# Amelie-Schreiber/ShapeMol

Measured on AMD Instinct MI355X. Metric: molecules/sec (1000-step DDPM sample, batch 256), higher is better.
Workload: dtype f32 (matrix operands split exactly into 3 x bf16 pieces = 24 bits, six piece products, fp32 accumulate); 1 GPU; BASELINE configs[1]: batch 256 MOSES-prior molecules (9-27 atoms) per GPU, 1000-step chain, fp32 results, k=8, synthetic shapes + hash-filled weights; besides the 5 warm-up steps an untimed 200-step chain runs first to reach the loaded clocks; batch_per_gpu=256, atoms_per_gpu=5541, total_atoms=5541, noise=device Philox, trajectories=kept in HBM, launch=hipGraph replay, parallelism=dp1 (whole batches per rank), ranks_seen=1

## Files before the change

### shapemol_amd/csrc/shapemol_hip.hip

```cpp
#include "../../include/shapemol_hip.h"
#include "sm_device.h"
#include "sm_edge.h"
#include "sm_edge_bf16.h"
#include "sm_edge16.h"
#include "sm_node.h"
#include "sm_node16.h"
#include "sm_edge_stream.h"
#include "sm_misc.h"
#include "sm_mesh.h"
#include "sm_guide_groups.h"
#include "sm_cfg.h"
#include "sm_mesh_groups.h"
#include <hip/hip_ext.h>

#include <algorithm>
#include <cmath>
#include <type_traits>
#include <cstdio>
#include <cstring>
#include <map>
#include <string>
#include <vector>

#include "sm_pack.h"

namespace {

#define HIPCHK(expr)                                                                         \
    do {                                                                                     \
        hipError_t e_ = (expr);                                                              \
        if (e_ != hipSuccess)                                                                \
            return fail(std::string(#expr) + ": " + hipGetErrorString(e_));                  \
    } while (0)

constexpr int kEdgeThreadsDefault = 768;
#ifndef SM_GRAPH_UNROLL
#define SM_GRAPH_UNROLL 20
#endif
constexpr int kGraphUnroll = SM_GRAPH_UNROLL;

struct ProfRec { const char *name; hipEvent_t e0, e1; };

enum class Guide { None, Cloud, Groups, Mesh, MeshGroups, Cfg };

}

struct shapemol_ctx {
    shapemol_config cfg{};
    int device = 0;
    int KP = 8;
    float *d_img = nullptr;
    float *ttab = nullptr;
    float *etab = nullptr;
    DevModel dm;
    int64_t capN = 0, capB = 0;
    std::vector<void *> allocs;
    int *mol_of = nullptr, *mol_off = nullptr, *t_mol = nullptr, *nbr = nullptr, *steps = nullptr;
    float *temb = nullptr, *inv = nullptr, *add0 = nullptr, *addp = nullptr, *ps = nullptr, *ew = nullptr;
    float *h_a = nullptr, *h_b = nullptr, *pre0 = nullptr, *preAB = nullptr, *q_x = nullptr, *q_h = nullptr, *att = nullptr, *o3 = nullptr, *pd = nullptr;
    ShapeTermArgs *prep_terms = nullptr; VnShapeArgs *prep_vn = nullptr; int n_prep_terms = 0;
    int2 *mol_span = nullptr;
    float *xsum = nullptr;
    float *part_rows = nullptr, *part_ms = nullptr;
    float *alpha = nullptr;
    float *x_a = nullptr, *x_b = nullptr, *x_state = nullptr, *pred_pos = nullptr, *pred_v = nullptr;
    int64_t *v_state = nullptr;
    unsigned long long *stamps = nullptr;
    unsigned long long *kstamps = nullptr;
    int kstamp_sel = -1;
    int stamp_on = 0;
    double *bn_acc = nullptr;
    int *status = nullptr;
    ChainParams *chain_params = nullptr;
    int64_t lastN = 0, lastB = 0;
    const float *last_h = nullptr, *last_x = nullptr;
    int stop_layer = -1, edge_threads = 0 , lin_waves = 16, edge_bf16 = 2, lin_bf16 = 1, chain_bf16 = 1, vn_fuse = 2;
    int vn_fold = 1;
    int max_mol_atoms = 0;
    int stream_whole_rounds = 0;
    int lin_fuse = 0;
    int bn_eval = 0;
    float *bn_run = nullptr;
    double *bn_eval_acc = nullptr;
    int ddpm_fold = 1;
    DdpmFold ddpm_vf{};
    int graph_fuse = 1;
// ... 445 lines not shown
               bool half_tiles, unsigned long long *stamps) {
    a.pre = pre; a.ld_pre = ld_pre; a.q = q; a.x = x; a.nbr = c->nbr; a.ew = c->ew; a.out = out; a.n_atoms = n_atoms; a.stamps = stamps;
    if (half_tiles) { a.out = c->part_rows; a.part_ms = c->part_ms; }
}

EdgeFusedArgs::VnFuse vn_fuse_args(const shapemol_ctx *c, int l, float *x_next, unsigned *arrive, int enable) {
    const DevLayer &D = c->dm.layer[l];
    const int hd = c->cfg.n_heads;
    return {c->ps + (size_t)l * c->capB * 2 * hd * 3, c->P(D.wf_x), c->P(D.wd_x), c->P(D.wf_o), c->P(D.wd_o), c->P(D.bn_g), c->P(D.bn_b),
            c->mol_of, c->pd, c->bn_acc + (size_t)l * kBnReplicas * 2 * hd, arrive, c->status + ST_VN_BARRIER, x_next, enable};
}

struct H2xPlan { EdgeFusedArgs::VnFuse vn{}; float *xsum = nullptr; VnFold pending{}; DdpmFold ddpm{}; bool stats_done = false, vn_done = false; };
H2xPlan h2x_plan(const shapemol_ctx *c, int l, bool fold, bool has_next, bool half_tiles, const double *stat_acc, const float *cur_x,
                 float *x_next, float *out_pos) {
    H2xPlan p;
    if (!c->vn_fuse || half_tiles) return p;
    const DevLayer &D = c->dm.layer[l];
    const int hd = c->cfg.n_heads;
    const double *acc = stat_acc + (size_t)l * kBnReplicas * 2 * hd;
    p.vn = vn_fuse_args(c, l, x_next, nullptr, 2);
    p.stats_done = true;
    const bool to_ddpm = !has_next && l == c->cfg.num_layers - 1 && out_pos && c->ddpm_fold && chain_guide(c) == Guide::None &&
                         c->cfg.num_classes <= 16 && hd <= 16;
    if (fold && has_next) p.pending = VnFold{c->pd, acc, c->P(D.bn_g), c->P(D.bn_b), c->xsum, cur_x, x_next, c->mol_span, c->status + ST_SPAN, 1};
    else if (fold && to_ddpm) p.ddpm = DdpmFold{c->pd, acc, c->P(D.bn_g), c->P(D.bn_b), c->xsum, cur_x, out_pos, hd, 1};
    else return p;
    p.xsum = c->xsum;
    p.vn_done = true;
    return p;
}

template <int H>
int run_score(shapemol_ctx *c, hipStream_t s, const float *x_in, const int64_t *v_in, int64_t N, int64_t B,
              bool sampling, int t_first, float *out_pos, float *out_h, float *out_v, bool reuse_graph = false) {
    const shapemol_config &g = c->cfg;
    const int L = g.num_layers, hd = g.n_heads, C = g.num_classes, D = g.time_emb_dim, KP = c->KP;
    const int n = (int)N;
    AtomEmbArgs ae{c->P(c->dm.embw), c->P(c->dm.embb), v_in, c->mol_of, c->ttab, c->t_mol, sampling ? c->steps : nullptr,
                   c->steps + 1, c->bn_acc, c->h_a, n, H, C, D, t_first, L * kBnReplicas * 2 * hd + L};
    const int nlay = c->stop_layer >= 0 ? std::min(c->stop_layer, L) : L;
    const bool fused_prologue = c->chain_bf16 && c->lin_bf16;
    if (fused_prologue) {
        const DevLayer &D0 = c->dm.layer[0];
        NodePrologueArgs pa{};
        pa.emb_wT = c->P(c->dm.embwT); pa.emb_b = ae.b; pa.v = v_in; pa.mol_of = c->mol_of; pa.ttab = c->ttab; pa.etab = c->etab; pa.t_mol = c->t_mol;
        pa.step_ptr = ae.step_ptr; pa.step_cur = ae.step_cur; pa.bn_acc = c->bn_acc; pa.h_out = c->h_a;
        pa.q = follow_of(c, D0.q_x2h, NODE_LN_RELU, c->q_x, H, H);
        pa.lin_img6 = c->P(c->node_f16 ? D0.pre16_x2h : D0.pre6_x2h); pa.add_mol = c->add0; pa.pre_out = c->pre0;
        pa.n_lin_tiles = nlay > 0 ? 4 * (H / 16) : 0; pa.ld_add = 4 * H; pa.ld_out = 4 * H;
        pa.n_atoms = n; pa.C = C; pa.D = D; pa.t_first = t_first; pa.bn_acc_len = ae.bn_acc_len;
        pa.stamps = c->kstamp_sel == 5 ? c->kstamps : nullptr;
        const int n_ct = (n + 15) / 16;
        if (c->node_f16 && c->feat_f16) LAUNCH("node_prologue", SMK((node_prologue16_kernel<H, true>), dim3((n_ct + CHAIN_COLS - 1) / CHAIN_COLS), dim3(H * 4),
                                                   2 * Chain16Lds<H>::FRAG * 16 + Chain16Lds<H>::PRE * 4, s, pa, c->status + ST_RANGE));
        else if (c->node_f16) LAUNCH("node_prologue", SMK(node_prologue16_kernel<H>, dim3((n_ct + CHAIN_COLS - 1) / CHAIN_COLS), dim3(H * 4),
                                                   2 * Chain16Lds<H>::FRAG * 16 + Chain16Lds<H>::PRE * 4, s, pa, c->status + ST_RANGE));
        else LAUNCH("node_prologue", SMK(node_prologue6_kernel<H>, dim3((n_ct + CHAIN_COLS - 1) / CHAIN_COLS), dim3(H * 4),
                                                   2 * Chain6Lds<H>::FRAG * 16 + Chain6Lds<H>::PRE * 4, s, pa));
    } else {
        LAUNCH("embed", SMK(atom_embed_kernel, dim3((N * H + 255) / 256), dim3(256), 0, s, ae));
    }
    const bool graph_fused = sampling && c->graph_fuse && c->max_mol_atoms > 0 && c->max_mol_atoms <= kGraphCap && KP <= 32 && c->n_pins == 0;
    if (reuse_graph) {
    } else if (graph_fused) {
        GraphArgs ga{x_in, c->mol_span, n, g.knn, KP, c->nbr, c->P(c->dm.ew.w1), c->P(c->dm.ew.b1), c->P(c->dm.ew.g), c->P(c->dm.ew.be),
                     c->P(c->dm.ew.w2), c->P(c->dm.ew.b2), c->ew, c->status + ST_SPAN, c->kstamp_sel == 4 ? c->kstamps : nullptr};
        const int apb = kGraphWaves * (KP >= 16 ? 1 : 16 / KP);
        DISPATCH_KP("graph", graph_kernel, (), dim3((n + apb - 1) / apb), dim3(kGraphWaves * 64), 0, s, ga);
    } else LAUNCH("knn", SMK(knn_kernel, dim3((N + 3) / 4), dim3(256), 0, s, x_in, c->mol_of, c->mol_off, n, g.knn, KP, c->nbr));
    if (sampling && c->n_pins > 0 && !reuse_graph)
        LAUNCH("knn", SMK(knn_pin_kernel, dim3(32), dim3(256), 0, s, c->pin_off, c->pin_steps, c->pin_atom, c->pin_nbr, c->pin_k, KP, c->steps + 1, n, c->nbr));
    EdgeWeightArgs ea{x_in, c->nbr, c->P(c->dm.ew.w1), c->P(c->dm.ew.b1), c->P(c->dm.ew.g), c->P(c->dm.ew.be),
                      c->P(c->dm.ew.w2), c->P(c->dm.ew.b2), c->ew, n * KP, KP};
    if (!graph_fused && !reuse_graph) {
        const int tiles = (n * KP + 15) / 16;
        LAUNCH("edge_weight", SMK(edge_weight_kernel<H>, dim3((tiles + 3) / 4), dim3(256), 0, s, ea));
    }
    const float *cur_x = x_in;
    float *cur_h = c->h_a;
    constexpr int NT = H / 16;
    bool v_done = false;
    if (nlay > 0 && !fused_prologue) {
        const DevLayer &D0 = c->dm.layer[0];
        if (launch_linear<H>(c, s, "node_pre", cur_h, c->P(D0.pre_x2h), c->P(D0.pre6_x2h), c->P(D0.pre16_x2h), c->add0, 4 * H, c->pre0, 4 * H, 4 * NT, n,
                             c->kstamp_sel == 0 ? c->kstamps : nullptr)) return 1;
        if (launch_mlp2<H, 1>(c, s, "node_q", D0.q_x2h, cur_h, nullptr, NODE_LN_RELU, nullptr, c->q_x, H, H, n)) return 1;
    }
    const bool fold = sampling && vn_fold_ok(c, n);
    double *stat_acc = c->bn_acc;
    if (c->bn_eval) {
        if (!c->bn_run) return fail("bn_eval = 1 needs the running statistics (shapemol_set_bn_running)");
// ... 181 lines not shown
    c->num_cu = prop.multiProcessorCount > 0 ? prop.multiProcessorCount : 256;

    Image im;
    if (build_model_image(*cfg, hm, im, c->dm, c->hid_max)) { delete c; return 1; }
    const DevModel &dm = c->dm;
    const int H = cfg->hidden_dim, T = cfg->num_timesteps;
    if (hipMalloc((void **)&c->d_img, im.d.size() * sizeof(float)) != hipSuccess) { delete c; return fail("hipMalloc(weights) failed"); }
    if (hipMemcpy(c->d_img, im.d.data(), im.d.size() * sizeof(float), hipMemcpyHostToDevice) != hipSuccess) { hipFree(c->d_img); delete c; return fail("hipMemcpy(weights) failed"); }
    if (H == 128 ? set_edge_attr<128>(c->KP) : set_edge_attr<32>(c->KP)) { hipFree(c->d_img); delete c; return 1; }
    {
        if (hipMalloc((void **)&c->ttab, (size_t)T * cfg->time_emb_dim * sizeof(float)) != hipSuccess) { hipFree(c->d_img); delete c; return fail("hipMalloc(time table) failed"); }
        TimeTableArgs ta{c->P(dm.te1w), c->P(dm.te1b), c->P(dm.te2w), c->P(dm.te2b), c->ttab, T, cfg->time_emb_dim};
        hipLaunchKernelGGL(time_table_kernel, dim3((T + 63) / 64), dim3(64), 0, nullptr, ta);
        if (hipDeviceSynchronize() != hipSuccess) { hipFree(c->ttab); hipFree(c->d_img); delete c; return fail("time table kernel failed"); }
        const int C = cfg->num_classes;
        if (hipMalloc((void **)&c->etab, (size_t)T * C * H * sizeof(float)) != hipSuccess) { hipFree(c->ttab); hipFree(c->d_img); delete c; return fail("hipMalloc(embedding table) failed"); }
        const int items = T * C * (H / 4);
        hipLaunchKernelGGL(emb_table_kernel, dim3((items + 255) / 256), dim3(256), 0, nullptr, c->P(dm.embwT), c->P(dm.embb), c->ttab, c->etab, T, C, cfg->time_emb_dim, H);
        if (hipDeviceSynchronize() != hipSuccess) { hipFree(c->etab); hipFree(c->ttab); hipFree(c->d_img); delete c; return fail("embedding table kernel failed"); }
    }
    *out = c;
    return 0;
}

void shapemol_destroy(shapemol_ctx *c) {
    if (!c) return;
    hipSetDevice(c->device);
    hipDeviceSynchronize();
    c->drop_graphs();
    for (auto &r : c->prof) { hipEventDestroy(r.e0); hipEventDestroy(r.e1); }
    for (void *p : c->allocs) hipFree(p);
    hipFree(c->ttab);
    hipFree(c->etab);
    hipFree(c->d_img);
    if (c->g_cloud) hipFree(c->g_cloud);
    if (c->gg_clouds) hipFree(c->gg_clouds);
    if (c->gg_table) hipFree(c->gg_table);
    if (c->m_faces) hipFree(c->m_faces);
    if (c->mg_faces) hipFree(c->mg_faces);
    if (c->m_within) hipFree(c->m_within);
    if (c->bn_run) hipFree(c->bn_run);
    if (c->bn_eval_acc) hipFree(c->bn_eval_acc);
    if (c->pin_off) { hipFree(c->pin_off); hipFree(c->pin_atom); hipFree(c->pin_nbr); }
    delete c;
}

int shapemol_set_bn_running(shapemol_ctx *c, const float *h_mean, const float *h_var, int64_t count) {
    if (!c || !h_mean || !h_var) return fail("shapemol_set_bn_running: null argument");
    const int L = c->cfg.num_layers, hd = c->cfg.n_heads;
    if (count != (int64_t)L * hd) return fail("shapemol_set_bn_running: count must be num_layers * n_heads");
    for (int64_t i = 0; i < count; ++i)
        if (!(h_var[i] >= 0.f) || !std::isfinite(h_mean[i]) || !std::isfinite(h_var[i])) return fail("shapemol_set_bn_running: statistics must be finite, variance >= 0");
    HIPCHK(hipSetDevice(c->device));
    HIPCHK(hipDeviceSynchronize());
    if (!c->bn_run) {
        HIPCHK(hipMalloc(&c->bn_run, 2 * count * sizeof(float)));
        HIPCHK(hipMalloc(&c->bn_eval_acc, (size_t)L * kBnReplicas * 2 * hd * sizeof(double)));
    }
    HIPCHK(hipMemcpy(c->bn_run, h_mean, count * sizeof(float), hipMemcpyHostToDevice));
    HIPCHK(hipMemcpy(c->bn_run + count, h_var, count * sizeof(float), hipMemcpyHostToDevice));
    return 0;
}

int shapemol_reserve(shapemol_ctx *c, int64_t max_atoms, int64_t max_mols) {
    if (!c || max_atoms < 1 || max_mols < 1) return fail("shapemol_reserve: bad argument");
    return ensure_workspace(c, max_atoms, max_mols);
}

int shapemol_score(shapemol_ctx *c, const float *d_pos, const int64_t *d_v, const int64_t *d_batch, int64_t N,
                   int64_t B, const float *d_shape, const int64_t *d_t, float *out_pos, float *out_h, float *out_v,
                   void *stream) {
    if (!c || !d_pos || !d_v || !d_batch || !d_shape || !d_t || !out_pos || !out_v) return fail("shapemol_score: null argument");
    if (N < 1 || B < 1 || N > (1 << 27)) return fail("shapemol_score: n_atoms / n_mols out of range");
    HIPCHK(hipSetDevice(c->device));
    if (ensure_workspace(c, N, B)) return 1;
    hipStream_t s = (hipStream_t)stream;
    c->lastN = N; c->lastB = B;
    HIPCHK(hipMemsetAsync(c->status, 0, 8 * sizeof(int), s));
    if (DISPATCH_H(c, run_prep<128>(c, s, d_batch, N, B, d_shape), run_prep<32>(c, s, d_batch, N, B, d_shape))) return 1;
    LAUNCH("prep", SMK(t_convert_kernel, dim3((B + 255) / 256), dim3(256), 0, s, d_t, (int)B, c->cfg.num_timesteps, c->t_mol, c->status));
    LAUNCH("prep", SMK(v_check_kernel, dim3((N + 255) / 256), dim3(256), 0, s, d_v, (int)N, c->cfg.num_classes, c->status));
    return DISPATCH_H(c, run_score<128>(c, s, d_pos, d_v, N, B, false, 0, out_pos, out_h, out_v),
                      run_score<32>(c, s, d_pos, d_v, N, B, false, 0, out_pos, out_h, out_v));
}

int shapemol_sample(shapemol_ctx *c, const float *d_init_pos, const int64_t *d_init_v, const int64_t *d_batch,
                    int64_t N, int64_t B, const float *d_shape, int32_t num_steps, const float *d_eps, const float *d_u,
                    uint64_t seed, const shapemol_traj *traj, float *out_pos, int64_t *out_v, int32_t use_graph, void *stream) {
    if (!c || !d_init_pos || !d_init_v || !d_batch || !d_shape || !out_pos || !out_v) return fail("shapemol_sample: null argument");
    if (N < 1 || B < 1 || N > (1 << 27)) return fail("shapemol_sample: n_atoms / n_mols out of range");
    if (num_steps < 1 || c->first_step + num_steps > c->cfg.num_timesteps) return fail("shapemol_sample: num_steps out of range");
    if ((d_eps == nullptr) != (d_u == nullptr)) return fail("shapemol_sample: d_eps and d_u must be given together");
    HIPCHK(hipSetDevice(c->device));
    if (ensure_workspace(c, N, B)) return 1;
    hipStream_t s = (hipStream_t)stream;
    c->lastN = N; c->lastB = B;
    const int t_first = c->cfg.num_timesteps - 1;
    const Guide kind = chain_guide(c);
    const bool mesh = kind == Guide::Mesh, mesh_groups = kind == Guide::MeshGroups, cfg = kind == Guide::Cfg;
    if (mesh && mesh_workspace(c, N, 1)) return 1;
    if (mesh_groups && mesh_workspace(c, N, c->mg_groups)) return 1;
    if (c->mg_groups > 0 && c->mg_mols != B)
        return fail("shapemol_sample: n_mols = " + std::to_string(B) + " but the mesh guidance groups cover " + std::to_string(c->mg_mols) + " molecules");
    if (c->gg_groups > 0 && c->gg_mols != B)
        return fail("shapemol_sample: n_mols = " + std::to_string(B) + " but the guidance groups cover " + std::to_string(c->gg_mols) + " molecules");
    if (kind == Guide::Groups && groups_table(c, s, d_batch, N, c->gg_ints, c->gg_groups)) return 1;
    if (mesh_groups && groups_table(c, s, d_batch, N, c->mg_ints, c->mg_groups)) return 1;
    HIPCHK(hipMemsetAsync(c->status, 0, 8 * sizeof(int), s));
    if (mesh) HIPCHK(hipMemsetAsync(c->m_cnt, 0, 4 * sizeof(int), s));
    if (mesh_groups && mesh_counters_clear(c, s, c->mg_groups)) return 1;
    if (DISPATCH_H(c, run_prep<128>(c, s, d_batch, N, B, d_shape), run_prep<32>(c, s, d_batch, N, B, d_shape))) return 1;
    if (cfg) {
        swap_uncond(c);
        const int rc = DISPATCH_H(c, run_prep_shape<128>(c, s, B, c->shape_zero), run_prep_shape<32>(c, s, B, c->shape_zero));
        swap_uncond(c);
        if (rc) return 1;
        HIPCHK(hipMemsetAsync(c->cfg_hist, 0, (size_t)2 * kCfgHistWords * sizeof(unsigned), s));
    }
    LAUNCH("prep", SMK(v_check_kernel, dim3((N + 255) / 256), dim3(256), 0, s, d_init_v, (int)N, c->cfg.num_classes, c->status));
    {
        ChainParams cp{};
        cp.seed = seed; cp.eps = d_eps; cp.u = d_u; cp.step_base = c->first_step; cp.guide_draws = mesh ? c->m_draws : (mesh_groups ? c->mg_draws : (c->gg_groups > 0 ? c->gg_draws : c->g_draws));
        if (traj) { cp.tr_pos = traj->pos_traj; cp.tr_v = traj->v_traj; cp.tr_v0 = traj->v0_traj; cp.tr_vt = traj->vt_traj;
                    cp.tr_pos_cond = traj->pos_cond_traj; cp.tr_v_cond = traj->v_cond_traj; }
        if (cfg) { cp.tr_pos_uncond = c->cfg_tr_pos_u; cp.tr_v_uncond = c->cfg_tr_v_u; }
        LAUNCH("prep", SMK(set_chain_params_kernel, dim3(1), dim3(1), 0, s, c->chain_params, cp, c->steps));
    }
    HIPCHK(hipMemcpyAsync(c->x_state, d_init_pos, N * 3 * sizeof(float), hipMemcpyDeviceToDevice, s));
    HIPCHK(hipMemcpyAsync(c->v_state, d_init_v, N * sizeof(int64_t), hipMemcpyDeviceToDevice, s));
// ... 65 lines not shown
int shapemol_set_option(shapemol_ctx *c, const char *name, int64_t value) {
    if (!c || !name) return fail("shapemol_set_option: null argument");
    const std::string k(name);
    if (k == "max_mol_atoms") {
        if (value < 0) return fail("max_mol_atoms must be >= 0");
        c->max_mol_atoms = (int)std::min<int64_t>(value, 1 << 20);
        return 0;
    }
    if (k == "first_step") {
        if (value < 0 || value >= c->cfg.num_timesteps) return fail("first_step must be in [0, num_timesteps)");
        c->first_step = (int)value;
        return 0;
    }
    if (k == "stop_layer") c->stop_layer = (int)value;
    else if (k == "edge_bf16") {
        if (value < 0 || value > 3) return fail("edge_bf16 must be 0 (fp32 MFMA), 1 (exactly split bf16, phase kernels), 2 (exactly split bf16, streaming kernels) or 3 (two-piece f16)");
        if (value != 3 && value != 2 && c->KP > 16) return fail("k > 16 runs on the streaming (edge_bf16 = 2) or the two-piece f16 (edge_bf16 = 3) edge kernels");
        if (value == 3 && c->hid_max > 6.0e4f) return fail("edge_bf16 = 3: the edge MLPs' LayerNorm outputs may exceed the fp16 range for these weights");
        c->edge_bf16 = (int)value;
    }
    else if (k == "edge_tiles") { if (value < -1 || value > 1) return fail("edge_tiles must be -1 (automatic), 0 (sliced one-job launches) or 1 (looping launch)"); c->edge_tiles = (int)value; }
    else if (k == "node_f16") c->node_f16 = value != 0;
    else if (k == "feat_f16") {
        if (value && (c->edge_bf16 != 3 || !c->node_f16)) return fail("feat_f16 = 1 needs the f16 kernels (edge_bf16 = 3, node_f16 = 1)");
        c->feat_f16 = value != 0;
    }
    else if (k == "lin_fuse") c->lin_fuse = value != 0;
    else if (k == "stream_whole_rounds") c->stream_whole_rounds = value != 0;
    else if (k == "x2h_chain") c->x2h_chain = value != 0;
    else if (k == "graph_fuse") c->graph_fuse = value != 0;
    else if (k == "bn_eval") c->bn_eval = value != 0;
    else if (k == "ddpm_fold") c->ddpm_fold = value != 0;
    else if (k == "vn_fold") c->vn_fold = value != 0;
    else if (k == "lin_bf16") c->lin_bf16 = (int)value;
    else if (k == "chain_bf16") c->chain_bf16 = (int)value;
    else if (k == "vn_fuse") c->vn_fuse = (int)value;
    else if (k == "lin_waves") { if (value < 1 || value > 16) return fail("lin_waves must be 1..16"); c->lin_waves = (int)value; }
    else if (k == "stamps") c->stamp_on = (int)value;
    else if (k == "kstamp_sel") c->kstamp_sel = (int)value;
    else if (k == "edge_waves") { if (value < 0 || value > 12) return fail("edge_waves must be 0 (automatic) .. 12"); c->edge_threads = (int)value * 64; }
    else return fail("unknown option " + k);
    hipSetDevice(c->device);
    c->drop_graphs();
    return 0;
}

int64_t shapemol_debug_read(shapemol_ctx *c, const char *name, void *dst, size_t max_bytes) {
    if (!c || !name || !dst) { fail("shapemol_debug_read: null argument"); return -1; }
    const std::string k(name);
    const shapemol_config &g = c->cfg;
    const int64_t N = c->lastN;
    const void *src = nullptr; size_t bytes = 0;
    int64_t dims[8] = {N, c->lastB, c->KP, g.hidden_dim, g.n_heads, g.num_layers, c->capN, c->capB};
    if (k == "dims") { if (max_bytes < sizeof(dims)) return -1; std::memcpy(dst, dims, sizeof(dims)); return sizeof(dims); }
    if (k == "captures") { if (max_bytes < 8) return -1; std::memcpy(dst, &c->n_captures, 8); return 8; }
    if (k == "nbr") { src = c->nbr; bytes = N * c->KP * 4; }
    else if (k == "ew") { src = c->ew; bytes = N * c->KP * 4; }
    else if (k == "h") { src = c->last_h; bytes = N * g.hidden_dim * 4; }
    else if (k == "x") { src = c->last_x; bytes = N * 3 * 4; }
    else if (k == "pre") { src = c->preAB; bytes = N * 8 * g.hidden_dim * 4; }
    else if (k == "q") { src = c->q_h; bytes = N * g.hidden_dim * 4; }
    else if (k == "att") { src = c->att; bytes = N * g.hidden_dim * 4; }
    else if (k == "o3") { src = c->o3; bytes = N * 48 * 4; }
    else if (k == "stamps") { src = c->stamps; bytes = 2048 * 8; }
    else if (k == "kstamps") { src = c->kstamps; bytes = (size_t)8 * 16 * 4096 * 8; }
    else if (k == "vn_err") { src = c->status + ST_VN_BARRIER; bytes = 4; }
    else if (k == "mesh_group_flags") { src = c->m_cnt ? c->m_cnt + 4 * c->m_cnt_cap : nullptr; bytes = (size_t)c->mg_flag_groups * 4; }
    else if (k == "cfg_stat") { src = c->cfg_stat; bytes = 2 * 4; }
    else if (k == "bnstat") { src = c->bn_acc; bytes = (size_t)g.num_layers * kBnReplicas * 2 * g.n_heads * 8; }
    else { fail("shapemol_debug_read: unknown buffer " + k); return -1; }
    if (!src || bytes > max_bytes) { fail("shapemol_debug_read: buffer unavailable or destination too small"); return -1; }
    if (hipSetDevice(c->device) != hipSuccess || hipDeviceSynchronize() != hipSuccess ||
        hipMemcpy(dst, src, bytes, hipMemcpyDeviceToHost) != hipSuccess) { fail("shapemol_debug_read: copy failed"); return -1; }
    return (int64_t)bytes;
}

void shapemol_debug_split_exact(float x, uint16_t *pieces) {
    uint16_t p[3];
    split3_host(x, p);
    pieces[0] = p[0]; pieces[1] = p[1]; pieces[2] = p[2];
}

int shapemol_set_knn_pins(shapemol_ctx *c, const int32_t *h_off, int32_t n_steps, const int32_t *h_atom, const int32_t *h_nbr, int64_t n_pins, int32_t k) {
    if (!c) return fail("shapemol_set_knn_pins: null context");
    HIPCHK(hipSetDevice(c->device));
    c->drop_graphs();
    HIPCHK(hipDeviceSynchronize());
    if (c->pin_off) { hipFree(c->pin_off); hipFree(c->pin_atom); hipFree(c->pin_nbr); c->pin_off = c->pin_atom = c->pin_nbr = nullptr; }
    c->n_pins = 0; c->pin_steps = 0; c->pin_k = 0;
    if (n_pins <= 0) return 0;
    if (!h_off || !h_atom || !h_nbr || n_steps < 1 || k < 1 || k > c->KP) return fail("shapemol_set_knn_pins: bad arguments");
    if (h_off[0] != 0 || h_off[n_steps] != n_pins) return fail("shapemol_set_knn_pins: offsets do not cover the pins");
// ... 92 lines not shown
```

### shapemol_amd/csrc/sm_misc.h

```cpp
#pragma once
#include "sm_device.h"
#include "sm_cfg.h"

enum StatusFlag { ST_VN_BARRIER = 0, ST_BATCH = 1, ST_ATOM_TYPE = 2, ST_TIME = 3, ST_RANGE = 4, ST_SPAN = 5, ST_MESH = 6 };

__global__ void mol_index_kernel(const int64_t *batch, int n, int n_mols, int *mol_of, int *mol_off, int *status) {
    const int i = blockIdx.x * blockDim.x + threadIdx.x;
    if (i >= n) return;
    const int64_t braw = batch[i], praw = i == 0 ? -1 : batch[i - 1];
    if (braw < 0 || braw >= n_mols || braw < praw) status[ST_BATCH] = 1;
    const int b = (int)min(max(braw, (int64_t)0), (int64_t)n_mols - 1);
    const int prev = (int)min(max(praw, (int64_t)-1), (int64_t)n_mols - 1);
    mol_of[i] = b;
    for (int m = prev + 1; m <= b; ++m) mol_off[m] = i;
    if (i == n - 1)
        for (int m = b + 1; m <= n_mols; ++m) mol_off[m] = n;
}

__global__ void mol_span_kernel(const int *mol_of, const int *mol_off, int n, int2 *span) {
    const int i = blockIdx.x * blockDim.x + threadIdx.x;
    if (i < n) span[i] = int2{mol_off[mol_of[i]], mol_off[mol_of[i] + 1]};
}

__global__ void t_convert_kernel(const int64_t *t, int n_mols, int n_timesteps, int *t_mol, int *status) {
// ... 184 lines not shown
    for (int k = 0; k < D; ++k) {
        const float4 wk = ldg4(emb_wT + (size_t)(C + k) * H + f);
        const float tk = te[k];
        y[0] += wk.x * tk; y[1] += wk.y * tk; y[2] += wk.z * tk; y[3] += wk.w * tk;
    }
    stg4(etab + ((size_t)t * C + v) * H + f, float4{y[0], y[1], y[2], y[3]});
}

struct AtomEmbArgs {
    const float *w, *b;
    const int64_t *v;
    const int *mol_of;
    const float *ttab;
    const int *t_mol;
    const int *step_ptr;
    int *step_cur;
    double *bn_acc;
    float *h;
    int n_atoms, H, C, D, t_first, bn_acc_len;
};
__global__ void atom_embed_kernel(AtomEmbArgs a) {
    const int idx = blockIdx.x * blockDim.x + threadIdx.x;
    const int step = a.step_ptr ? *a.step_ptr : 0;
    if (idx == 0 && a.step_ptr) *a.step_cur = step;
    for (int i = idx; i < a.bn_acc_len; i += gridDim.x * blockDim.x) a.bn_acc[i] = 0.0;
    if (idx >= a.n_atoms * a.H) return;
    const int i = idx / a.H, f = idx % a.H, ld = a.C + a.D;
    const int t = a.step_ptr ? a.t_first - step : a.t_mol[a.mol_of[i]];
    const float *w = a.w + (size_t)f * ld;
    float y = a.b[f] + w[min(max((int)a.v[i], 0), a.C - 1)];
    const float *te = a.ttab + (size_t)t * a.D;
    for (int k = 0; k < a.D; ++k) y += w[a.C + k] * te[k];
    a.h[idx] = y;
}

SM_DEV float dist2_rounded(float dx, float dy, float dz) {
#pragma clang fp contract(off)
    const float a = dx * dx, b = dy * dy, c = dz * dz;
    return (a + b) + c;
}

__global__ void knn_kernel(const float *x, const int *mol_of, const int *mol_off, int n_atoms, int k,
                           int kp, int *nbr) {
    const int lane = threadIdx.x & 63;
    const int i = blockIdx.x * (blockDim.x >> 6) + (threadIdx.x >> 6);
    if (i >= n_atoms) return;
    const int m = mol_of[i], s = mol_off[m], cnt = mol_off[m + 1] - s;
    const float xi = x[i * 3], yi = x[i * 3 + 1], zi = x[i * 3 + 2];
    const int deg = min(k, cnt - 1);
    for (int c = lane; c < cnt; c += 64) {
        const int j = s + c;
        if (j == i) continue;
        float dx = x[j * 3] - xi, dy = x[j * 3 + 1] - yi, dz = x[j * 3 + 2] - zi;
        const float dc = dist2_rounded(dx, dy, dz);
        int rank = 0;
        for (int o = 0; o < cnt; ++o) {
            const int jo = s + o;
            dx = x[jo * 3] - xi; dy = x[jo * 3 + 1] - yi; dz = x[jo * 3 + 2] - zi;
            const float d_o = dist2_rounded(dx, dy, dz);
            rank += (jo != i) && (o != c) && (d_o < dc || (d_o == dc && o < c));
        }
        if (rank < k) nbr[(size_t)i * kp + rank] = j;
    }
    for (int sl = lane; sl < kp; sl += 64)
        if (sl >= deg) nbr[(size_t)i * kp + sl] = -1;
}
// ... 679 lines not shown
```

### shapemol_amd/csrc/sm_node.h

```cpp
#pragma once
#include "sm_device.h"

enum NodeMode { NODE_LN_RELU = 1, NODE_SSP = 2 };
constexpr int kNodeThreads = 1024;

struct NodeLinArgs {
    const float *in;
    const float *wimg;
    const float *add_mol;
    const int *mol_of;
    float *out;
    int n_atoms, n_out_tiles, tiles_per_group;
    int ld_add, ld_out;
    unsigned long long *stamps;
    int nwave;
};

constexpr int kLinChunk = 8;

template <int H>
__global__ void __launch_bounds__(kNodeThreads)
node_linear_kernel(NodeLinArgs a) {
    constexpr int NT = H / 16;
    constexpr int XS = H + 16;
// ... 706 lines not shown
        const int fa = 32 * sb + 4 * (sl >> 4);
        float vv[8];
        {
            const float *row = a.etab + ((size_t)t * a.C + vi) * H + fa;
            const float4 r0 = ldg4(row), r1 = ldg4(row + 16);
            vv[0] = r0.x; vv[1] = r0.y; vv[2] = r0.z; vv[3] = r0.w; vv[4] = r1.x; vv[5] = r1.y; vv[6] = r1.z; vv[7] = r1.w;
        }
        if (at_raw < a.n_atoms) {
            stg4(a.h_out + (size_t)at * H + fa, float4{vv[0], vv[1], vv[2], vv[3]});
            stg4(a.h_out + (size_t)at * H + fa + 16, float4{vv[4], vv[5], vv[6], vv[7]});
        }
        u32x4 hi, mid, lo;
        split3_bf16(vv, hi, mid, lo);
        u32x4 *dst = fh + (sb * CC + sc) * 64 + frag_slot(sb, sl);
        dst[0] = hi; dst[NB * CC * 64] = mid; dst[2 * NB * CC * 64] = lo;
    }
    if (a.n_lin_tiles > 0) load_w(a.lin_img6, ot, wl);
    const float4 b1 = ldg4(a.q.b1 + f0);
    __syncthreads();

    {
        f32x4 acc[CC];
#pragma unroll
        for (int c = 0; c < CC; ++c) acc[c] = f32x4{b1.x, b1.y, b1.z, b1.w};
        gemm6(wq1, fh, acc);
#pragma unroll
        for (int c = 0; c < CC; ++c) stg4(pre0 + (c * 16 + n) * XS + f0, float4{acc[c][0], acc[c][1], acc[c][2], acc[c][3]});
    }
    const bool onq = ot < a.q.nt2;
    if (onq) load_w(a.q.w2img6, ot, wq1);
    auto lin_tile = [&](int tile, const u32x4 (&w)[3][NB]) {
        f32x4 acc[CC];
#pragma unroll
        for (int c = 0; c < CC; ++c) {
            const float4 t = a.add_mol ? ldg4(a.add_mol + (size_t)a.mol_of[atom_of(c)] * a.ld_add + 16 * tile + 4 * g)
                                       : float4{0.f, 0.f, 0.f, 0.f};
            acc[c] = f32x4{t.x, t.y, t.z, t.w};
        }
        gemm6(w, fh, acc);
#pragma unroll
        for (int c = 0; c < CC; ++c)
            if (atom_ok(c)) stg4(a.pre_out + (size_t)atom_of(c) * a.ld_out + 16 * tile + 4 * g, float4{acc[c][0], acc[c][1], acc[c][2], acc[c][3]});
    };
    for (int tile = ot; tile < a.n_lin_tiles; tile += 2 * NT) {
        u32x4 wn[3][NB];
        const bool more1 = tile + NT < a.n_lin_tiles, more2 = tile + 2 * NT < a.n_lin_tiles;
        if (more1) load_w(a.lin_img6, tile + NT, wn);
        lin_tile(tile, wl);
        if (more2) load_w(a.lin_img6, tile + 2 * NT, wl);
        if (more1) lin_tile(tile + NT, wn);
    }
    __syncthreads();
    {
        const int col = ot * (64 / LPC) + lane / LPC, ln = lane % LPC;
        const int b = ln >> 2, gg = ln & 3;
        const int fa = 32 * b + 4 * gg;
        const float4 p0 = ldg4(pre0 + col * XS + fa), p1 = ldg4(pre0 + col * XS + fa + 16);
        float v[8] = {p0.x, p0.y, p0.z, p0.w, p1.x, p1.y, p1.z, p1.w};
        float s = 0.f;
#pragma unroll
        for (int i = 0; i < 8; ++i) s += v[i];
        const float mean = seg_sum<LPC>(s) * (1.0f / H);
        float q = 0.f;
#pragma unroll
        for (int i = 0; i < 8; ++i) { const float d = v[i] - mean; q += d * d; }
        const float var = seg_sum<LPC>(q) * (1.0f / H);
        const float rstd = 1.0f / sqrtf(var + 1e-5f);
        const float4 g0 = ldg4(a.q.ln_g + fa), g1 = ldg4(a.q.ln_g + fa + 16), e0 = ldg4(a.q.ln_b + fa), e1 = ldg4(a.q.ln_b + fa + 16);
        const float ga[8] = {g0.x, g0.y, g0.z, g0.w, g1.x, g1.y, g1.z, g1.w};
        const float be[8] = {e0.x, e0.y, e0.z, e0.w, e1.x, e1.y, e1.z, e1.w};
#pragma unroll
        for (int i = 0; i < 8; ++i) v[i] = fmaxf((v[i] - mean) * rstd * ga[i] + be[i], 0.f);
// ... 18 lines not shown
```

### shapemol_amd/csrc/sm_node16.h

```cpp
#pragma once
#include "sm_node.h"
#include "sm_edge16.h"

SM_DEV void split2_8(const float (&v)[8], u32x4 &hi, u32x4 &lo, int *range_flag) {
    float m = 0.f;
#pragma unroll
    for (int q = 0; q < 4; ++q) {
        unsigned h, l;
        split2_pair(v[2 * q], v[2 * q + 1], h, l);
        hi[q] = h; lo[q] = l;
        m = fmaxf(m, fmaxf(fabsf(v[2 * q]), fabsf(v[2 * q + 1])));
    }
    if (!(m < 6.0e4f)) *range_flag = 1;
}

constexpr int kLin16Chunk = 12;

template <int H, bool P1 = false>
__global__ void __launch_bounds__(kNodeThreads)
node_linear16_kernel(NodeLinArgs a, int *range_flag) {
    constexpr int NB = H / 32;
    extern __shared__ __attribute__((aligned(16))) unsigned char lin16_lds[];
    u32x4 *frag = reinterpret_cast<u32x4 *>(lin16_lds);
    const int lane = threadIdx.x & 63, wave = threadIdx.x >> 6;
// ... 409 lines not shown
                const float tk = te[k];
                y[0] += wk.x * tk; y[1] += wk.y * tk; y[2] += wk.z * tk; y[3] += wk.w * tk;
            }
#pragma unroll
            for (int j = 0; j < 4; ++j) vv[4 * hf + j] = y[j];
        }
        if (at_raw < a.n_atoms) {
            stg4(a.h_out + (size_t)at * H + fa, float4{vv[0], vv[1], vv[2], vv[3]});
            stg4(a.h_out + (size_t)at * H + fa + 16, float4{vv[4], vv[5], vv[6], vv[7]});
        }
        u32x4 hi, lo;
        split2_8(vv, hi, lo, range_flag);
        u32x4 *dst = fh + (sb * CC + sc) * 64 + frag_slot(sb, sl);
        dst[0] = hi; dst[NB * CC * 64] = lo;
    }
    if (a.n_lin_tiles > 0) N16::template load_w<NB>(a.lin_img6, ot, lane, wl);
    const float4 b1 = ldg4(a.q.b1 + f0);
    SM_TICK(a.stamps, 1);
    __syncthreads();
    SM_TICK(a.stamps, 2);

    {
        f32x4 acc[CC];
#pragma unroll
        for (int c = 0; c < CC; ++c) acc[c] = f32x4{b1.x, b1.y, b1.z, b1.w};
        N16::template gemm<NB>(wq1, fh, acc, lane);
        N16::store_pre(pre0, acc, n, f0);
    }
    const bool onq = ot < a.q.nt2;
    if (onq) N16::template load_w<NB>(a.q.w2img6, ot, lane, wq1);
    auto lin_tile = [&](int tile, const u32x4 (&w)[2][NB]) {
        f32x4 acc[CC];
#pragma unroll
        for (int c = 0; c < CC; ++c) {
            const float4 t = a.add_mol ? ldg4(a.add_mol + (size_t)a.mol_of[atom_of(c)] * a.ld_add + 16 * tile + 4 * g)
                                       : float4{0.f, 0.f, 0.f, 0.f};
            acc[c] = f32x4{t.x, t.y, t.z, t.w};
        }
        N16::template gemm<NB>(w, fh, acc, lane);
#pragma unroll
        for (int c = 0; c < CC; ++c)
            if (atom_ok(c)) stg4(a.pre_out + (size_t)atom_of(c) * a.ld_out + 16 * tile + 4 * g, float4{acc[c][0], acc[c][1], acc[c][2], acc[c][3]});
    };
    for (int tile = ot; tile < a.n_lin_tiles; tile += 2 * NT) {
        u32x4 wn[2][NB];
        const bool more1 = tile + NT < a.n_lin_tiles, more2 = tile + 2 * NT < a.n_lin_tiles;
        if (more1) N16::template load_w<NB>(a.lin_img6, tile + NT, lane, wn);
        lin_tile(tile, wl);
        if (more2) N16::template load_w<NB>(a.lin_img6, tile + 2 * NT, lane, wl);
        if (more1) lin_tile(tile + NT, wn);
    }
    SM_TICK(a.stamps, 3);
    __syncthreads();
    SM_TICK(a.stamps, 4);
    N16::normalise(pre0, NODE_LN_RELU, a.q.ln_g, a.q.ln_b, fhid, ot, lane, range_flag);
    __syncthreads();
    SM_TICK(a.stamps, 5);
    if (onq) {
        const float4 b = ldg4(a.q.b2 + f0);
        f32x4 acc[CC];
#pragma unroll
        for (int c = 0; c < CC; ++c) acc[c] = f32x4{b.x, b.y, b.z, b.w};
        N16::template gemm<NB>(wq1, fhid, acc, lane);
#pragma unroll
        for (int c = 0; c < CC; ++c)
            if (atom_ok(c)) stg4(a.q.out + (size_t)atom_of(c) * a.q.ld_out + f0, float4{acc[c][0], acc[c][1], acc[c][2], acc[c][3]});
    }
    SM_STAMP(a.stamps, 6);
}
```

Baseline: 367.6 molecules/s.

## Precompute node prologue outputs per (timestep, atom type) into lookup tables

The node prologue (embedding, first-layer q MLP and the x2h linear) depends only on the timestep and atom class, plus a per-molecule additive term. The outputs are now precomputed once for every (t, class) row, and each step becomes a gather from these tables plus the per-molecule add, in place of the GEMM-heavy prologue kernel. The linear tile is reordered so the molecule add comes after the GEMM, which lets the tabulated pre-activations match exactly. This costs table memory of T*C*5*H floats and a one-time build.

```diff
diff --git a/shapemol_amd/csrc/shapemol_hip.hip b/shapemol_amd/csrc/shapemol_hip.hip
--- a/shapemol_amd/csrc/shapemol_hip.hip
+++ b/shapemol_amd/csrc/shapemol_hip.hip
@@ -52,6 +52,11 @@
     float *d_img = nullptr;
     float *ttab = nullptr;
     float *etab = nullptr;
+    float *q_tab = nullptr;
+    float *pre_tab = nullptr;
+    int64_t *tab_v = nullptr; int *tab_mol_of = nullptr, *tab_t_mol = nullptr, *tab_flag = nullptr;
+    int tab_key = 0;
+    int prologue_tab = 1;
     DevModel dm;
     int64_t capN = 0, capB = 0;
     std::vector<void *> allocs;
@@ -563,6 +568,53 @@
 }
 
 template <int H>
+NodePrologueArgs prologue_args(const shapemol_ctx *c, const int64_t *v, const int *mol_of, const int *t_mol, const float *add_mol,
+                               float *h_out, float *q_out, float *pre_out, int n) {
+    const DevLayer &D0 = c->dm.layer[0];
+    NodePrologueArgs pa{};
+    pa.emb_wT = c->P(c->dm.embwT); pa.emb_b = c->P(c->dm.embb); pa.v = v; pa.mol_of = mol_of; pa.ttab = c->ttab; pa.etab = c->etab; pa.t_mol = t_mol;
+    pa.h_out = h_out;
+    pa.q = follow_of(c, D0.q_x2h, NODE_LN_RELU, q_out, H, H);
+    pa.lin_img6 = c->P(c->node_f16 ? D0.pre16_x2h : D0.pre6_x2h); pa.add_mol = add_mol; pa.pre_out = pre_out;
+    pa.n_lin_tiles = 4 * (H / 16); pa.ld_add = 4 * H; pa.ld_out = 4 * H;
+    pa.n_atoms = n; pa.C = c->cfg.num_classes; pa.D = c->cfg.time_emb_dim;
+    return pa;
+}
+
+template <int H>
+int launch_prologue(shapemol_ctx *c, hipStream_t s, const NodePrologueArgs &pa, int *range_flag = nullptr) {
+    const int n_ct = (pa.n_atoms + 15) / 16;
+    const dim3 grid((n_ct + CHAIN_COLS - 1) / CHAIN_COLS), block(H * 4);
+    if (!range_flag) range_flag = c->status + ST_RANGE;
+    if (c->node_f16 && c->feat_f16) LAUNCH("node_prologue", SMK((node_prologue16_kernel<H, true>), grid, block, 2 * Chain16Lds<H>::FRAG * 16 + Chain16Lds<H>::PRE * 4, s, pa, range_flag));
+    else if (c->node_f16) LAUNCH("node_prologue", SMK(node_prologue16_kernel<H>, grid, block, 2 * Chain16Lds<H>::FRAG * 16 + Chain16Lds<H>::PRE * 4, s, pa, range_flag));
+    else LAUNCH("node_prologue", SMK(node_prologue6_kernel<H>, grid, block, 2 * Chain6Lds<H>::FRAG * 16 + Chain6Lds<H>::PRE * 4, s, pa));
+    return 0;
+}
+
+int prologue_tab_key(const shapemol_ctx *c) { return 1 + (c->node_f16 ? 1 + (c->feat_f16 ? 1 : 0) : 0); }
+
+template <int H>
+int ensure_prologue_tables(shapemol_ctx *c, hipStream_t s) {
+    if (!c->prologue_tab || !(c->chain_bf16 && c->lin_bf16) || c->tab_key == prologue_tab_key(c)) return 0;
+    const int T = c->cfg.num_timesteps, C = c->cfg.num_classes;
+    const size_t rows = (size_t)T * C;
+    if (!c->q_tab) {
+        void *blk = nullptr;
+        HIPCHK(hipMalloc(&blk, rows * 5 * H * sizeof(float) + rows * (sizeof(int64_t) + sizeof(int)) + ((size_t)T + 1) * sizeof(int)));
+        c->q_tab = static_cast<float *>(blk); c->pre_tab = c->q_tab + rows * H;
+        c->tab_v = reinterpret_cast<int64_t *>(c->pre_tab + rows * 4 * H);
+        c->tab_mol_of = reinterpret_cast<int *>(c->tab_v + rows); c->tab_t_mol = c->tab_mol_of + rows; c->tab_flag = c->tab_t_mol + T;
+    }
+    c->tab_key = 0;
+    LAUNCH("prep", SMK(prologue_tab_index_kernel, dim3((unsigned)((rows + 255) / 256)), dim3(256), 0, s, c->tab_v, c->tab_mol_of, c->tab_t_mol, c->tab_flag, T, C));
+    const NodePrologueArgs pa = prologue_args<H>(c, c->tab_v, c->tab_mol_of, c->tab_t_mol, nullptr, c->etab, c->q_tab, c->pre_tab, (int)rows);
+    if (launch_prologue<H>(c, s, pa, c->tab_flag)) return 1;
+    c->tab_key = prologue_tab_key(c);
+    return 0;
+}
+
+template <int H>
 int run_score(shapemol_ctx *c, hipStream_t s, const float *x_in, const int64_t *v_in, int64_t N, int64_t B,
               bool sampling, int t_first, float *out_pos, float *out_h, float *out_v, bool reuse_graph = false) {
     const shapemol_config &g = c->cfg;
@@ -572,23 +624,17 @@
                    c->steps + 1, c->bn_acc, c->h_a, n, H, C, D, t_first, L * kBnReplicas * 2 * hd + L};
     const int nlay = c->stop_layer >= 0 ? std::min(c->stop_layer, L) : L;
     const bool fused_prologue = c->chain_bf16 && c->lin_bf16;
-    if (fused_prologue) {
-        const DevLayer &D0 = c->dm.layer[0];
-        NodePrologueArgs pa{};
-        pa.emb_wT = c->P(c->dm.embwT); pa.emb_b = ae.b; pa.v = v_in; pa.mol_of = c->mol_of; pa.ttab = c->ttab; pa.etab = c->etab; pa.t_mol = c->t_mol;
-        pa.step_ptr = ae.step_ptr; pa.step_cur = ae.step_cur; pa.bn_acc = c->bn_acc; pa.h_out = c->h_a;
-        pa.q = follow_of(c, D0.q_x2h, NODE_LN_RELU, c->q_x, H, H);
-        pa.lin_img6 = c->P(c->node_f16 ? D0.pre16_x2h : D0.pre6_x2h); pa.add_mol = c->add0; pa.pre_out = c->pre0;
-        pa.n_lin_tiles = nlay > 0 ? 4 * (H / 16) : 0; pa.ld_add = 4 * H; pa.ld_out = 4 * H;
-        pa.n_atoms = n; pa.C = C; pa.D = D; pa.t_first = t_first; pa.bn_acc_len = ae.bn_acc_len;
+    if (fused_prologue && c->prologue_tab) {
+        if (c->tab_key != prologue_tab_key(c)) return fail("run_score: the prologue tables are not built for this precision mode");
+        PrologueTabArgs ta{c->etab, c->q_tab, c->pre_tab, c->tab_flag, v_in, c->mol_of, c->t_mol, ae.step_ptr, ae.step_cur, c->bn_acc,
+                           c->add0, c->h_a, c->q_x, c->pre0, c->status + ST_RANGE, n, C, g.num_timesteps, t_first, ae.bn_acc_len};
+        LAUNCH("node_prologue", SMK(node_prologue_tab_kernel<H>, dim3((unsigned)((N * 16 + kProTabThreads - 1) / kProTabThreads)), dim3(kProTabThreads), 0, s, ta));
+    } else if (fused_prologue) {
+        NodePrologueArgs pa = prologue_args<H>(c, v_in, c->mol_of, c->t_mol, c->add0, c->h_a, c->q_x, c->pre0, n);
+        pa.step_ptr = ae.step_ptr; pa.step_cur = ae.step_cur; pa.bn_acc = c->bn_acc; pa.bn_acc_len = ae.bn_acc_len; pa.t_first = t_first;
+        if (nlay == 0) pa.n_lin_tiles = 0;
         pa.stamps = c->kstamp_sel == 5 ? c->kstamps : nullptr;
-        const int n_ct = (n + 15) / 16;
-        if (c->node_f16 && c->feat_f16) LAUNCH("node_prologue", SMK((node_prologue16_kernel<H, true>), dim3((n_ct + CHAIN_COLS - 1) / CHAIN_COLS), dim3(H * 4),
-                                                   2 * Chain16Lds<H>::FRAG * 16 + Chain16Lds<H>::PRE * 4, s, pa, c->status + ST_RANGE));
-        else if (c->node_f16) LAUNCH("node_prologue", SMK(node_prologue16_kernel<H>, dim3((n_ct + CHAIN_COLS - 1) / CHAIN_COLS), dim3(H * 4),
-                                                   2 * Chain16Lds<H>::FRAG * 16 + Chain16Lds<H>::PRE * 4, s, pa, c->status + ST_RANGE));
-        else LAUNCH("node_prologue", SMK(node_prologue6_kernel<H>, dim3((n_ct + CHAIN_COLS - 1) / CHAIN_COLS), dim3(H * 4),
-                                                   2 * Chain6Lds<H>::FRAG * 16 + Chain6Lds<H>::PRE * 4, s, pa));
+        if (launch_prologue<H>(c, s, pa)) return 1;
     } else {
         LAUNCH("embed", SMK(atom_embed_kernel, dim3((N * H + 255) / 256), dim3(256), 0, s, ae));
     }
@@ -836,6 +882,7 @@
     for (void *p : c->allocs) hipFree(p);
     hipFree(c->ttab);
     hipFree(c->etab);
+    hipFree(c->q_tab);
     hipFree(c->d_img);
     if (c->g_cloud) hipFree(c->g_cloud);
     if (c->gg_clouds) hipFree(c->gg_clouds);
@@ -880,6 +927,7 @@
     if (ensure_workspace(c, N, B)) return 1;
     hipStream_t s = (hipStream_t)stream;
     c->lastN = N; c->lastB = B;
+    if (DISPATCH_H(c, ensure_prologue_tables<128>(c, s), ensure_prologue_tables<32>(c, s))) return 1;
     HIPCHK(hipMemsetAsync(c->status, 0, 8 * sizeof(int), s));
     if (DISPATCH_H(c, run_prep<128>(c, s, d_batch, N, B, d_shape), run_prep<32>(c, s, d_batch, N, B, d_shape))) return 1;
     LAUNCH("prep", SMK(t_convert_kernel, dim3((B + 255) / 256), dim3(256), 0, s, d_t, (int)B, c->cfg.num_timesteps, c->t_mol, c->status));
@@ -899,6 +947,7 @@
     if (ensure_workspace(c, N, B)) return 1;
     hipStream_t s = (hipStream_t)stream;
     c->lastN = N; c->lastB = B;
+    if (DISPATCH_H(c, ensure_prologue_tables<128>(c, s), ensure_prologue_tables<32>(c, s))) return 1;
     const int t_first = c->cfg.num_timesteps - 1;
     const Guide kind = chain_guide(c);
     const bool mesh = kind == Guide::Mesh, mesh_groups = kind == Guide::MeshGroups, cfg = kind == Guide::Cfg;
@@ -1030,6 +1079,7 @@
     else if (k == "bn_eval") c->bn_eval = value != 0;
     else if (k == "ddpm_fold") c->ddpm_fold = value != 0;
     else if (k == "vn_fold") c->vn_fold = value != 0;
+    else if (k == "prologue_tab") c->prologue_tab = value != 0;
     else if (k == "lin_bf16") c->lin_bf16 = (int)value;
     else if (k == "chain_bf16") c->chain_bf16 = (int)value;
     else if (k == "vn_fuse") c->vn_fuse = (int)value;
@@ -1056,6 +1106,10 @@
     else if (k == "ew") { src = c->ew; bytes = N * c->KP * 4; }
     else if (k == "h") { src = c->last_h; bytes = N * g.hidden_dim * 4; }
     else if (k == "x") { src = c->last_x; bytes = N * 3 * 4; }
+    else if (k == "h0") { src = c->h_a; bytes = N * g.hidden_dim * 4; }
+    else if (k == "q_x") { src = c->q_x; bytes = N * g.hidden_dim * 4; }
+    else if (k == "pre0") { src = c->pre0; bytes = N * 4 * g.hidden_dim * 4; }
+    else if (k == "add0") { src = c->add0; bytes = (size_t)c->lastB * 4 * g.hidden_dim * 4; }
     else if (k == "pre") { src = c->preAB; bytes = N * 8 * g.hidden_dim * 4; }
     else if (k == "q") { src = c->q_h; bytes = N * g.hidden_dim * 4; }
     else if (k == "att") { src = c->att; bytes = N * g.hidden_dim * 4; }
diff --git a/shapemol_amd/csrc/sm_misc.h b/shapemol_amd/csrc/sm_misc.h
--- a/shapemol_amd/csrc/sm_misc.h
+++ b/shapemol_amd/csrc/sm_misc.h
@@ -240,6 +240,80 @@
     const float *te = a.ttab + (size_t)t * a.D;
     for (int k = 0; k < a.D; ++k) y += w[a.C + k] * te[k];
     a.h[idx] = y;
+}
+
+struct PrologueTabArgs {
+    const float *etab, *q_tab, *pre_tab;
+    const int *tab_flag;
+    const int64_t *v;
+    const int *mol_of;
+    const int *t_mol;
+    const int *step_ptr;
+    int *step_cur;
+    double *bn_acc;
+    const float *add_mol;
+    float *h_out, *q_out, *pre_out;
+    int *range_flag;
+    int n_atoms, C, T, t_first, bn_acc_len;
+};
+
+constexpr int kProTabThreads = 256;
+
+template <int H>
+__global__ void __launch_bounds__(kProTabThreads)
+node_prologue_tab_kernel(PrologueTabArgs a) {
+    constexpr int R = H / 64;
+    static_assert(H % 64 == 0 || H == 32, "16 lanes x 16 bytes cover a row in whole passes");
+    const int gid = blockIdx.x * kProTabThreads + threadIdx.x;
+    const int step = a.step_ptr ? *a.step_ptr : 0;
+    if (gid == 0) {
+        if (a.step_ptr) *a.step_cur = step;
+        if (*a.tab_flag) *a.range_flag = 1;
+    }
+    for (int i = gid; i < a.bn_acc_len; i += gridDim.x * kProTabThreads) a.bn_acc[i] = 0.0;
+    const int atom = gid >> 4, ln = gid & 15;
+    if (atom >= a.n_atoms) return;
+    const int mol = a.mol_of[atom];
+    const int t = min(max(a.step_ptr ? a.t_first - step : a.t_mol[mol], 0), a.T - 1);
+    const int vi = min(max((int)a.v[atom], 0), a.C - 1);
+    const size_t row = (size_t)t * a.C + vi;
+    if constexpr (H == 32) {
+        const int f = 4 * (ln & 7);
+        const float *src = (ln < 8 ? a.etab : a.q_tab) + row * H + f;
+        const float4 hq = ldg4(src);
+        const float4 p0 = ldg4(a.pre_tab + row * 4 * H + 4 * ln), p1 = ldg4(a.pre_tab + row * 4 * H + 64 + 4 * ln);
+        const float4 m0 = ldg4(a.add_mol + (size_t)mol * 4 * H + 4 * ln), m1 = ldg4(a.add_mol + (size_t)mol * 4 * H + 64 + 4 * ln);
+        stg4((ln < 8 ? a.h_out : a.q_out) + (size_t)atom * H + f, hq);
+        stg4(a.pre_out + (size_t)atom * 4 * H + 4 * ln, float4{p0.x + m0.x, p0.y + m0.y, p0.z + m0.z, p0.w + m0.w});
+        stg4(a.pre_out + (size_t)atom * 4 * H + 64 + 4 * ln, float4{p1.x + m1.x, p1.y + m1.y, p1.z + m1.z, p1.w + m1.w});
+    } else {
+        float4 h[R], q[R], p[4 * R], m[4 * R];
+#pragma unroll
+        for (int r = 0; r < R; ++r) {
+            h[r] = ldg4(a.etab + row * H + 64 * r + 4 * ln);
+            q[r] = ldg4(a.q_tab + row * H + 64 * r + 4 * ln);
+        }
+#pragma unroll
+        for (int r = 0; r < 4 * R; ++r) {
+            p[r] = ldg4(a.pre_tab + row * 4 * H + 64 * r + 4 * ln);
+            m[r] = ldg4(a.add_mol + (size_t)mol * 4 * H + 64 * r + 4 * ln);
+        }
+#pragma unroll
+        for (int r = 0; r < R; ++r) {
+            stg4(a.h_out + (size_t)atom * H + 64 * r + 4 * ln, h[r]);
+            stg4(a.q_out + (size_t)atom * H + 64 * r + 4 * ln, q[r]);
+        }
+#pragma unroll
+        for (int r = 0; r < 4 * R; ++r)
+            stg4(a.pre_out + (size_t)atom * 4 * H + 64 * r + 4 * ln, float4{p[r].x + m[r].x, p[r].y + m[r].y, p[r].z + m[r].z, p[r].w + m[r].w});
+    }
+}
+
+__global__ void prologue_tab_index_kernel(int64_t *v, int *mol_of, int *t_mol, int *flag, int T, int C) {
+    const int i = blockIdx.x * blockDim.x + threadIdx.x;
+    if (i == 0) *flag = 0;
+    if (i < T) t_mol[i] = i;
+    if (i < T * C) { v[i] = i % C; mol_of[i] = i / C; }
 }
 
 SM_DEV float dist2_rounded(float dx, float dy, float dz) {
diff --git a/shapemol_amd/csrc/sm_node.h b/shapemol_amd/csrc/sm_node.h
--- a/shapemol_amd/csrc/sm_node.h
+++ b/shapemol_amd/csrc/sm_node.h
@@ -762,12 +762,14 @@
     auto lin_tile = [&](int tile, const u32x4 (&w)[3][NB]) {
         f32x4 acc[CC];
 #pragma unroll
+        for (int c = 0; c < CC; ++c) acc[c] = f32x4{0.f, 0.f, 0.f, 0.f};
+        gemm6(w, fh, acc);
+#pragma unroll
         for (int c = 0; c < CC; ++c) {
-            const float4 t = a.add_mol ? ldg4(a.add_mol + (size_t)a.mol_of[atom_of(c)] * a.ld_add + 16 * tile + 4 * g)
-                                       : float4{0.f, 0.f, 0.f, 0.f};
-            acc[c] = f32x4{t.x, t.y, t.z, t.w};
-        }
-        gemm6(w, fh, acc);
+            if (!a.add_mol) continue;
+            const float4 t = ldg4(a.add_mol + (size_t)a.mol_of[atom_of(c)] * a.ld_add + 16 * tile + 4 * g);
+            acc[c][0] += t.x; acc[c][1] += t.y; acc[c][2] += t.z; acc[c][3] += t.w;
+        }
 #pragma unroll
         for (int c = 0; c < CC; ++c)
             if (atom_ok(c)) stg4(a.pre_out + (size_t)atom_of(c) * a.ld_out + 16 * tile + 4 * g, float4{acc[c][0], acc[c][1], acc[c][2], acc[c][3]});
diff --git a/shapemol_amd/csrc/sm_node16.h b/shapemol_amd/csrc/sm_node16.h
--- a/shapemol_amd/csrc/sm_node16.h
+++ b/shapemol_amd/csrc/sm_node16.h
@@ -465,12 +465,14 @@
     auto lin_tile = [&](int tile, const u32x4 (&w)[2][NB]) {
         f32x4 acc[CC];
 #pragma unroll
+        for (int c = 0; c < CC; ++c) acc[c] = f32x4{0.f, 0.f, 0.f, 0.f};
+        N16::template gemm<NB>(w, fh, acc, lane);
+#pragma unroll
         for (int c = 0; c < CC; ++c) {
-            const float4 t = a.add_mol ? ldg4(a.add_mol + (size_t)a.mol_of[atom_of(c)] * a.ld_add + 16 * tile + 4 * g)
-                                       : float4{0.f, 0.f, 0.f, 0.f};
-            acc[c] = f32x4{t.x, t.y, t.z, t.w};
-        }
-        N16::template gemm<NB>(w, fh, acc, lane);
+            if (!a.add_mol) continue;
+            const float4 t = ldg4(a.add_mol + (size_t)a.mol_of[atom_of(c)] * a.ld_add + 16 * tile + 4 * g);
+            acc[c][0] += t.x; acc[c][1] += t.y; acc[c][2] += t.z; acc[c][3] += t.w;
+        }
 #pragma unroll
         for (int c = 0; c < CC; ++c)
             if (atom_ok(c)) stg4(a.pre_out + (size_t)atom_of(c) * a.ld_out + 16 * tile + 4 * g, float4{acc[c][0], acc[c][1], acc[c][2], acc[c][3]});
```

Result: faster. 376.8 molecules/s, median of 6 (+2.5%).
